# sash-a/CleanRL.jl

Hardware: NVIDIA B200
Metric: ppo_env_steps_per_sec (higher is better)
Workload: dtype f32

## Files before the change

### cleanrl.jl_b200/csrc/rollout.cu

```cuda
#include "kernels.h"
#include "mlp_tile.cuh"

namespace {

constexpr int RE = 32;
constexpr int ROLL_FWD = CRL_THREADS;
constexpr int ROLL_THREADS = ROLL_FWD + 64;
constexpr int BIG_FWD = 128, BIG_THREADS = BIG_FWD + 64;
constexpr int BAR_FWD = 1, BAR_SPEC = 2, BAR_BOOK = 3;

__device__ __forceinline__ void nbar_sync(int id, int n) { asm volatile("bar.sync %0, %1;" ::"r"(id), "r"(n) : "memory"); }
__device__ __forceinline__ void nbar_arrive(int id, int n) { asm volatile("bar.arrive %0, %1;" ::"r"(id), "r"(n) : "memory"); }

template <int ENV> struct RolloutSmem {
  using G = TileGeom<4, 2>;
  using E = EnvTraits<ENV>;
  static constexpr int SP = G::S_PAD;
  static constexpr int PARAMS = 0;
  static constexpr int X = PARAMS + SmemParams<ENV>::SIZE;
  static constexpr int H1 = X + CRL_MAXD * SP;
  static constexpr int H2 = H1 + G::ROWS * SP;
  static constexpr int OUT = H2 + G::ROWS * SP;
  static constexpr int ST = OUT + 4 * RE;
  static constexpr int SPEC = ST + 4 * RE;
  static constexpr int RST = SPEC + 2 * 4 * RE;
  static constexpr int NOISE = RST + 4 * RE;
  static constexpr int USED = NOISE + 2 * RE;
  static constexpr int BOOK = USED + RE;
  static constexpr int FLOATS = BOOK + 4 * RE;
  static constexpr size_t BYTES = FLOATS * sizeof(float);
  static_assert((NOISE % 2) == 0, "the Float64 uniforms need 8-byte alignment");
};

#ifdef ROLL_TRACE
#define RTR(i) do { if (tr) tr[i] = clock64(); } while (0)
#else
#define RTR(i) do { } while (0)
#endif

template <int ENV> struct HeadRow { float w[CRL_H]; float b; };
template <int ENV> __device__ __forceinline__ void load_head_row(const float* sp, HeadRow<ENV>& hr) {
  using E = EnvTraits<ENV>;
  const int o = threadIdx.x / RE;
#pragma unroll
  for (int k = 0; k < CRL_H; k++) hr.w[k] = 0.0f;
  hr.b = 0.0f;
  if (threadIdx.x >= RE * (E::A + 1)) return;
  if (o < E::A) {
    const float* a = sp + SmemParams<ENV>::ACTOR;
#pragma unroll
    for (int k = 0; k < CRL_H; k++) hr.w[k] = a[NetOff<E::D, E::A>::W3 + k * E::A + o];
    hr.b = a[NetOff<E::D, E::A>::B3 + o];
  } else {
    const float* c = sp + SmemParams<ENV>::CRITIC;
#pragma unroll
    for (int k = 0; k < CRL_H; k++) hr.w[k] = c[NetOff<E::D, 1>::W3 + k];
    hr.b = c[NetOff<E::D, 1>::B3];
  }
}

template <int ENV, bool BOOKSYNC = false>
__device__ __forceinline__ void forward32(const ThreadCoord<TileGeom<4, 2>>& tc, float* smem, const HeadRow<ENV>& hr,
                                          long long* tr = nullptr) {
  using G = TileGeom<4, 2>;
  using E = EnvTraits<ENV>;
  using SM = RolloutSmem<ENV>;
  constexpr int SP = G::S_PAD;
  float* sp = smem + SM::PARAMS;
  float* xs = smem + SM::X;
  float* h1 = smem + SM::H1;
  float* h2 = smem + SM::H2;
  float* so = smem + SM::OUT;
  const float* np = sp + net_base<ENV>(tc.net);
  using NO = NetOff<E::D, 1>;
  RTR(0);
  tile_layer_fwd4<G, E::D>(tc, np + NO::W1, np + NO::B1, xs, h1 + tc.net * CRL_H * SP);
  RTR(1);
  nbar_sync(BAR_FWD, ROLL_FWD);
  RTR(2);
  tile_layer_fwd4<G, CRL_H>(tc, np + NO::W2, np + NO::B2, h1 + tc.net * CRL_H * SP, h2 + tc.net * CRL_H * SP);
  RTR(3);
  nbar_sync(BAR_FWD, ROLL_FWD);
  RTR(4);
  if (threadIdx.x < RE * (E::A + 1)) {
    const int o = threadIdx.x / RE, e = threadIdx.x % RE;
    const float* hrow = h2 + (o < E::A ? 0 : CRL_H) * SP + e;
    float hv[CRL_H];
#pragma unroll
    for (int k = 0; k < CRL_H; k++) hv[k] = hrow[k * SP];
    if (BOOKSYNC) nbar_sync(BAR_BOOK, RE * (E::A + 1) + 32);
    float acc = 0.0f;
#pragma unroll
    for (int k = 0; k < CRL_H; k++) acc = fmaf(hr.w[k], hv[k], acc);
    acc += hr.b;
    so[o * RE + e] = acc;
  }
  RTR(5);
  nbar_sync(BAR_FWD, ROLL_FWD);
  RTR(6);
}

struct FwdCoord8x4 {
  int q, p, net, nb;
  __device__ FwdCoord8x4() {
    const int lane = threadIdx.x & 31, w = (threadIdx.x >> 5) & 3;
    q = w * 4 + (lane >> 3);
    p = lane & 7;
    net = q >> 3;
    nb = 8 * (q & 7);
  }
};
template <int K>
__device__ __forceinline__ void fwd_layer_8x4(const FwdCoord8x4& fc, const float* __restrict__ Wt, const float* __restrict__ bias,
                                              const float* __restrict__ in, float* __restrict__ out) {
  constexpr int SP = RE + 4, PF = 2;
  const float* wp = Wt + fc.nb;
  const float* ap = in + 4 * fc.p;
  const float4 b0 = *reinterpret_cast<const float4*>(bias + fc.nb), b1 = *reinterpret_cast<const float4*>(bias + fc.nb + 4);
  float2 acc[8][2];
#pragma unroll
  for (int j = 0; j < 8; j++) acc[j][0] = acc[j][1] = make_float2(0.0f, 0.0f);
  float4 w0[PF], w1[PF], av[PF];
#pragma unroll
  for (int i = 0; i < PF; i++) {
    if (i < K) {
      w0[i] = *reinterpret_cast<const float4*>(wp + i * CRL_H);
      w1[i] = *reinterpret_cast<const float4*>(wp + i * CRL_H + 4);
      av[i] = *reinterpret_cast<const float4*>(ap + i * SP);
    }
  }
#pragma unroll
  for (int k0 = 0; k0 < K; k0 += PF) {
    float4 w0n[PF], w1n[PF], avn[PF];
#pragma unroll
    for (int i = 0; i < PF; i++) {
      if (k0 + PF + i < K) {
        w0n[i] = *reinterpret_cast<const float4*>(wp + (k0 + PF + i) * CRL_H);
        w1n[i] = *reinterpret_cast<const float4*>(wp + (k0 + PF + i) * CRL_H + 4);
        avn[i] = *reinterpret_cast<const float4*>(ap + (k0 + PF + i) * SP);
      }
    }
#pragma unroll
    for (int i = 0; i < PF; i++) {
      if (k0 + i < K) {
        const float2 a01 = make_float2(av[i].x, av[i].y), a23 = make_float2(av[i].z, av[i].w);
#pragma unroll
        for (int j = 0; j < 8; j++) {
          const float wj = j < 4 ? f4_get(w0[i], j) : f4_get(w1[i], j - 4);
          const float2 ww = make_float2(wj, wj);
          acc[j][0] = __ffma2_rn(ww, a01, acc[j][0]);
          acc[j][1] = __ffma2_rn(ww, a23, acc[j][1]);
        }
      }
    }
#pragma unroll
    for (int i = 0; i < PF; i++) { w0[i] = w0n[i]; w1[i] = w1n[i]; av[i] = avn[i]; }
  }
#pragma unroll
  for (int j = 0; j < 8; j++) {
    const float b = j < 4 ? f4_get(b0, j) : f4_get(b1, j - 4);
    const float2 t0 = tanh_fast2(__fadd2_rn(acc[j][0], make_float2(b, b)));
    const float2 t1 = tanh_fast2(__fadd2_rn(acc[j][1], make_float2(b, b)));
    *reinterpret_cast<float4*>(out + (fc.nb + j) * SP + 4 * fc.p) = make_float4(t0.x, t0.y, t1.x, t1.y);
  }
}
template <int ENV>
__device__ __forceinline__ void forward32_big(const FwdCoord8x4& fc, float* smem) {
  using E = EnvTraits<ENV>;
  using SM = RolloutSmem<ENV>;
  constexpr int SP = RE + 4;
  static_assert(SP == TileGeom<4, 2>::S_PAD, "both forward variants share one activation layout");
  float* sp = smem + SM::PARAMS;
  float* xs = smem + SM::X;
  float* h1 = smem + SM::H1;
  float* h2 = smem + SM::H2;
  float* so = smem + SM::OUT;
  const float* np = sp + net_base<ENV>(fc.net);
  using NO = NetOff<E::D, 1>;
  fwd_layer_8x4<E::D>(fc, np + NO::W1, np + NO::B1, xs, h1 + fc.net * CRL_H * SP);
  nbar_sync(BAR_FWD, BIG_FWD);
  fwd_layer_8x4<CRL_H>(fc, np + NO::W2, np + NO::B2, h1 + fc.net * CRL_H * SP, h2 + fc.net * CRL_H * SP);
  nbar_sync(BAR_FWD, BIG_FWD);
  if (threadIdx.x < RE * (E::A + 1)) {
    const int o = threadIdx.x / RE, e = threadIdx.x % RE;
    const float* hrow = h2 + (o < E::A ? 0 : CRL_H) * SP + e;
    nbar_sync(BAR_BOOK, RE * (E::A + 1) + 32);
    float acc = 0.0f;
    if (o < E::A) {
      const float* a = sp + SmemParams<ENV>::ACTOR;
#pragma unroll 16
      for (int k = 0; k < CRL_H; k++) acc = fmaf(a[NetOff<E::D, E::A>::W3 + k * E::A + o], hrow[k * SP], acc);
      acc += a[NetOff<E::D, E::A>::B3 + o];
    } else {
      const float* c = sp + SmemParams<ENV>::CRITIC;
#pragma unroll 16
      for (int k = 0; k < CRL_H; k++) acc = fmaf(c[NetOff<E::D, 1>::W3 + k], hrow[k * SP], acc);
      acc += c[NetOff<E::D, 1>::B3];
    }
    so[o * RE + e] = acc;
  }
  nbar_sync(BAR_FWD, BIG_FWD);
}

template <int ENV, bool BIG>
__global__ void __launch_bounds__(BIG ? BIG_THREADS : ROLL_THREADS, BIG ? 2 : 1) rollout_kernel(RolloutArgs a) {
  constexpr int FWD = BIG ? BIG_FWD : ROLL_FWD;
  constexpr int SW0 = FWD / 32;
  using G = TileGeom<4, 2>;
  using E = EnvTraits<ENV>;
  using SM = RolloutSmem<ENV>;
  constexpr int SP = G::S_PAD;
  constexpr int D = E::D, A = E::A, S = E::S;
  constexpr bool CART = ENV == CRL_ENV_CARTPOLE;
  extern __shared__ __align__(16) float smem[];
  float* sp = smem + SM::PARAMS;
  float* xs = smem + SM::X;
  float* so = smem + SM::OUT;
  float* st_s = smem + SM::ST;
  float* spec_s = smem + SM::SPEC;
  float* rst_s = smem + SM::RST;
  double* noise_d = reinterpret_cast<double*>(smem + SM::NOISE);
  float* noise_f = smem + SM::NOISE;
  int* used_s = reinterpret_cast<int*>(smem + SM::USED);
  int* act_s = reinterpret_cast<int*>(smem + SM::BOOK);
  float* actf_s = smem + SM::BOOK + RE;
  float* rew_s = smem + SM::BOOK + 2 * RE;
  int* done_s = reinterpret_cast<int*>(smem + SM::BOOK + 3 * RE);
  const ThreadCoord<G> tc;
  const FwdCoord8x4 fc;

  load_params<ENV>(a.params, sp);
  for (int i = threadIdx.x; i < CRL_MAXD * SP; i += blockDim.x) xs[i] = 0.0f;

  const int warp = threadIdx.x >> 5;
  const int e = threadIdx.x & 31;
  const long long n = (long long)blockIdx.x * RE + e;
  const bool fwd = threadIdx.x < FWD;
  const bool owner = threadIdx.x < RE;
  const bool booker = warp == SW0 + 1;
  const bool in_range = n < a.N;
  const bool valid = owner && in_range;
  const unsigned long long step0 = a.ds->policy_step;
  const uint32_t gid = (uint32_t)(a.env_id_base + (int)n);

  float st[S];
  float obs[D];
  int env_t = 0;
  uint32_t resets = 0;
  bool done_flag = false;
  int ep_len = 0;
  double ep_ret = 0.0;
  bool prev_done = false;
  float obs_b[D];
  unsigned long long agg_n = 0;
  double agg_ret = 0.0, agg_len = 0.0, agg_max = -INFINITY;
  bool rec_pending = false;
  unsigned int rec_slot = 0;
  crl_episode rec;
  rec.step = 0; rec.env = 0; rec.length = 0; rec._pad = 0; rec.episode_return = 0.0;

#pragma unroll
  for (int i = 0; i < S; i++) st[i] = 0.0f;
#pragma unroll
  for (int k = 0; k < D; k++) obs_b[k] = 0.0f;
  if (valid) {
#pragma unroll
    for (int i = 0; i < S; i++) st[i] = a.env_state[n * S + i];
    env_t = a.env_t[n];
    resets = a.reset_count[n];
  }
  if (booker && in_range) {
    ep_len = a.ep_length[n];
    ep_ret = a.ep_return[n];
    resets = a.reset_count[n];
  }
  __syncthreads();
  HeadRow<ENV> hr;
  if (!BIG) load_head_row<ENV>(sp, hr);
  if (owner) {
    env_obs<ENV>(st, obs);
#pragma unroll
    for (int k = 0; k < D; k++) xs[k * SP + e] = obs[k];
#pragma unroll
    for (int i = 0; i < S; i++) st_s[i * RE + e] = st[i];
    used_s[e] = 0;
  }
  auto prepare_reset = [&]() {
    float u4[4], rs[S];
    int rt;
    rng_reset_uniforms(a.seed, gid, resets, u4);
    env_reset<ENV>(rs, rt, u4);
#pragma unroll
    for (int i = 0; i < S; i++) rst_s[i * RE + e] = rs[i];
  };
  if (booker && !a.reset_noise) prepare_reset();

  auto book = [&](int tb, const float (&zv)[A + 1], int act_i, float act_f, float r, bool dn) {
    const long long b = (long long)tb * a.N + n;
    ep_len += 1;
    float logprob;
    if (!E::CONT) {
      float m = zv[0];
#pragma unroll
      for (int k = 1; k < A; k++) m = fmaxf(m, zv[k]);
      float sum = 0.0f;
#pragma unroll
      for (int k = 0; k < A; k++) sum = __fadd_rn(sum, expf(__fsub_rn(zv[k], m)));
      const float ls = logf(sum);
      logprob = __fsub_rn(__fsub_rn(zv[0], m), ls);
#pragma unroll
      for (int k = 1; k < A; k++) logprob = (act_i == k) ? __fsub_rn(__fsub_rn(zv[k], m), ls) : logprob;
    } else {
      float lps = 0.0f;
#pragma unroll
      for (int k = 0; k < A; k++) {
        const float mean = zv[k];
        const float logstd = sp[SmemParams<ENV>::LOGSTD + k];
        const float sd = expf(logstd);
        const float diff = __fsub_rn(act_f, mean);
        const float q = __fdiv_rn(-__fmul_rn(diff, diff), __fmul_rn(__fmul_rn(2.0f, sd), sd));
        lps = __fadd_rn(lps, __fsub_rn(__fsub_rn(q, logstd), 0.9189385332046727f));
      }
      logprob = lps;
    }
    if (rec_pending) {
      if (rec_slot < (unsigned int)a.ep_capacity) a.records[rec_slot] = rec;
      rec_pending = false;
    }
    ep_ret += (double)r;
    if (in_range) {
      if (D == 4) {
        reinterpret_cast<float4*>(a.state)[b] = make_float4(obs_b[0], obs_b[1], obs_b[2], obs_b[3]);
      } else {
#pragma unroll
        for (int k = 0; k < D; k++) a.state[b * D + k] = obs_b[k];
      }
      if (!E::CONT) reinterpret_cast<int32_t*>(a.action)[b] = act_i;
      else reinterpret_cast<float*>(a.action)[b * A] = act_f;
      a.logprob[b] = logprob;
      a.value[b] = zv[A];
      a.terminal[b] = prev_done ? 1 : 0;
      a.reward[b] = r;
      if (dn) {
        rec_slot = atomicAdd(&a.eb->count, 1u);
        rec_pending = true;
        rec.step = tb; rec.env = (int)n; rec.length = ep_len; rec._pad = 0; rec.episode_return = ep_ret;
        agg_n += 1; agg_ret += ep_ret; agg_len += (double)ep_len; agg_max = fmax(agg_max, ep_ret);
        ep_ret = 0.0;
        ep_len = 0;
      }
    }
    prev_done = dn;
  };
  static_assert(!E::CONT || A == 1, "the Gaussian head hands one action per env to the bookkeeping warp");
  __syncthreads();

  for (int t = 0; t < a.T; t++) {
    if (!fwd) {
      if (booker) {
        float zv[A + 1];
#pragma unroll
        for (int k = 0; k <= A; k++) zv[k] = so[k * RE + e];
        const int act_i = act_s[e];
        const float act_f = actf_s[e], r = rew_s[e];
        const bool dn = done_s[e] != 0;
        nbar_arrive(BAR_BOOK, RE * (A + 1) + 32);
        if (t > 0) book(t - 1, zv, act_i, act_f, r, dn);
#pragma unroll
        for (int k = 0; k < D; k++) obs_b[k] = xs[k * SP + e];
        if (!a.reset_noise && used_s[e]) {
          resets += 1;
          prepare_reset();
          used_s[e] = 0;
        }
      }
      if (warp == SW0 && !a.action_noise) {
        if (!E::CONT) {
          noise_d[e] = in_range ? rng_action_uniform(a.seed, gid, step0 + (unsigned long long)t) : 0.0;
        } else {
          float zn[2] = {0.0f, 0.0f};
          if (in_range) rng_action_normals(a.seed, gid, step0 + (unsigned long long)t, zn);
          noise_f[e] = zn[0];
          noise_f[RE + e] = zn[1];
        }
      }
      if (CART) {
        float s4[4];
#pragma unroll
        for (int i = 0; i < 4; i++) s4[i] = st_s[i * RE + e];
        cartpole_dynamics(s4, warp - SW0);
#pragma unroll
        for (int i = 0; i < 4; i++) spec_s[((warp - SW0) * 4 + i) * RE + e] = s4[i];
      }
      __threadfence_block();
      nbar_arrive(BAR_SPEC, RE + 64);
    } else {
      if (BIG) forward32_big<ENV>(fc, smem); else forward32<ENV, true>(tc, smem, hr);
      if (owner) {
        const long long b = (long long)t * a.N + n;
        int act_i = 0;
        float act_f = 0.0f;
        if (!E::CONT) {
          float z[A], p[A];
#pragma unroll
          for (int k = 0; k < A; k++) z[k] = so[k * RE + e];
          float m = z[0];
#pragma unroll
          for (int k = 1; k < A; k++) m = fmaxf(m, z[k]);
          float ex[A], sum = 0.0f;
#pragma unroll
          for (int k = 0; k < A; k++) { ex[k] = expf(__fsub_rn(z[k], m)); sum = __fadd_rn(sum, ex[k]); }
          float psum = 0.0f;
#pragma unroll
          for (int k = 0; k < A; k++) {
            p[k] = __fdiv_rn(ex[k], sum);
            psum = __fadd_rn(psum, p[k]);
          }
          nbar_sync(BAR_SPEC, RE + 64);
          double u = 0.0;
          if (valid) u = a.action_noise ? a.action_noise[b] : noise_d[e];
          const double tt = __dmul_rn(u, (double)psum);
          float cw = p[0];
          int i = 0;
#pragma unroll
          for (int k = 1; k < A; k++) {
            if ((double)cw < tt && i == k - 1) { i = k; cw = __fadd_rn(cw, p[k]); }
          }
          act_i = i;
        } else {
          nbar_sync(BAR_SPEC, RE + 64);
          float zn = 0.0f;
          if (valid) zn = a.action_noise ? (float)a.action_noise[b * A] : noise_f[e];
          const float mean = so[e];
          const float sd = expf(sp[SmemParams<ENV>::LOGSTD]);
          act_f = __fadd_rn(mean, __fmul_rn(sd, zn));
        }
        float r;
        bool dn;
        if (CART) {
#pragma unroll
          for (int i = 0; i < 4; i++) st[i] = spec_s[(act_i * 4 + i) * RE + e];
          env_t += 1;
          cartpole_outcome(st, env_t, a.max_steps, r, dn);
        } else {
          pendulum_step(st, env_t, act_f, a.max_steps, r, dn);
        }
        env_obs<ENV>(st, obs);
        done_flag = dn;
        act_s[e] = act_i; actf_s[e] = act_f; rew_s[e] = r; done_s[e] = dn ? 1 : 0;
        if (valid && dn) {
          if (a.reset_noise) {
            const float4 v = reinterpret_cast<const float4*>(a.reset_noise)[b];
            const float u4[4] = {v.x, v.y, v.z, v.w};
            env_reset<ENV>(st, env_t, u4);
          } else {
#pragma unroll
            for (int i = 0; i < S; i++) st[i] = rst_s[i * RE + e];
            env_t = 0;
            used_s[e] = 1;
          }
          resets += 1;
          if (a.fresh_obs_after_reset) env_obs<ENV>(st, obs);
        }
#pragma unroll
        for (int k = 0; k < D; k++) xs[k * SP + e] = obs[k];
#pragma unroll
        for (int i = 0; i < S; i++) st_s[i * RE + e] = st[i];
      }
    }
    __syncthreads();
  }
  if (!fwd) {
    if (booker) {
      float zv[A + 1];
#pragma unroll
      for (int k = 0; k <= A; k++) zv[k] = so[k * RE + e];
      const int act_i = act_s[e];
      const float act_f = actf_s[e], r = rew_s[e];
      const bool dn = done_s[e] != 0;
      nbar_arrive(BAR_BOOK, RE * (A + 1) + 32);
      book(a.T - 1, zv, act_i, act_f, r, dn);
      if (rec_pending && rec_slot < (unsigned int)a.ep_capacity) a.records[rec_slot] = rec;
      if (in_range) {
        a.ep_length[n] = ep_len;
        a.ep_return[n] = ep_ret;
      }
      const double sr = warp_sum(agg_ret), sl = warp_sum(agg_len), mx = warp_max(agg_max);
      unsigned long long cn = agg_n;
#pragma unroll
      for (int o = 16; o > 0; o >>= 1) cn += __shfl_xor_sync(0xffffffffu, cn, o);
      if (e == 0 && cn > 0) {
        atomicAdd(&a.eb->n_episodes, cn);
        atomicAdd(&a.eb->sum_return, sr);
        atomicAdd(&a.eb->sum_length, sl);
        unsigned long long* addr = reinterpret_cast<unsigned long long*>(&a.eb->max_return);
        unsigned long long old = *addr, assumed;
        do {
          assumed = old;
          if (__longlong_as_double((long long)assumed) >= mx) break;
          old = atomicCAS(addr, assumed, (unsigned long long)__double_as_longlong(mx));
        } while (assumed != old);
      }
    }
    return;
  }

  float obs_last[D];
#pragma unroll
  for (int k = 0; k < D; k++) obs_last[k] = obs[k];
  if (owner) {
    float fresh[D];
    env_obs<ENV>(st, fresh);
#pragma unroll
    for (int k = 0; k < D; k++) xs[k * SP + e] = fresh[k];
  }
  nbar_sync(BAR_FWD, FWD);
  if (BIG) forward32_big<ENV>(fc, smem); else forward32<ENV, true>(tc, smem, hr);
  if (valid) {
    a.next_value[n] = so[A * RE + e];
#pragma unroll
    for (int i = 0; i < S; i++) a.env_state[n * S + i] = st[i];
    a.env_t[n] = env_t;
    a.reset_count[n] = resets;
#pragma unroll
    for (int k = 0; k < D; k++) a.next_obs[n * D + k] = obs_last[k];
    a.next_done[n] = done_flag ? 1 : 0;
  }
}

template <int ENV>
__global__ void env_step_raw_kernel(float* state, int* t, const void* action, float* reward, uint8_t* done,
                                    long long n, int max_steps) {
  constexpr int S = EnvTraits<ENV>::S;
  const long long i = (long long)blockIdx.x * blockDim.x + threadIdx.x;
  if (i >= n) return;
  float st[S];
#pragma unroll
  for (int k = 0; k < S; k++) st[k] = state[i * S + k];
  int tt = t[i];
  float r;
  bool dn;
  if (ENV == CRL_ENV_CARTPOLE) cartpole_step(st, tt, reinterpret_cast<const int32_t*>(action)[i], max_steps, r, dn);
  else pendulum_step(st, tt, reinterpret_cast<const float*>(action)[i], max_steps, r, dn);
#pragma unroll
  for (int k = 0; k < S; k++) state[i * S + k] = st[k];
  t[i] = tt;
  reward[i] = r;
  done[i] = dn ? 1 : 0;
}

template <int ENV>
__global__ void __launch_bounds__(CRL_THREADS) policy_forward_raw_kernel(const float* params, const float* obs,
                                                                         float* out_policy, float* logp,
                                                                         float* value, long long n) {
  using G = TileGeom<4, 2>;
  using E = EnvTraits<ENV>;
  using SM = RolloutSmem<ENV>;
  constexpr int SP = G::S_PAD;
  constexpr int D = E::D, A = E::A;
  extern __shared__ __align__(16) float smem[];
  float* xs = smem + SM::X;
  float* so = smem + SM::OUT;
  const ThreadCoord<G> tc;
  load_params<ENV>(params, smem + SM::PARAMS);
  const int e = threadIdx.x;
  const long long i = (long long)blockIdx.x * RE + e;
  if (e < RE) {
#pragma unroll
    for (int k = 0; k < D; k++) xs[k * SP + e] = i < n ? obs[i * D + k] : 0.0f;
  }
  __syncthreads();
  HeadRow<ENV> hr;
  load_head_row<ENV>(smem + SM::PARAMS, hr);
  forward32<ENV>(tc, smem, hr);
  if (e < RE && i < n) {
    float z[A];
#pragma unroll
    for (int k = 0; k < A; k++) { z[k] = so[k * RE + e]; out_policy[i * A + k] = z[k]; }
    value[i] = so[A * RE + e];
    if (!E::CONT) {
      float m = z[0];
#pragma unroll
      for (int k = 1; k < A; k++) m = fmaxf(m, z[k]);
      float sum = 0.0f;
#pragma unroll
      for (int k = 0; k < A; k++) sum = __fadd_rn(sum, expf(__fsub_rn(z[k], m)));
      const float ls = logf(sum);
#pragma unroll
      for (int k = 0; k < A; k++) logp[i * A + k] = __fsub_rn(__fsub_rn(z[k], m), ls);
    }
  }
}

template <int ENV> cudaError_t launch_rollout_t(const RolloutArgs& a, cudaStream_t s) {
  const int grid = (a.N + RE - 1) / RE;
  static int sms = 0;
  if (sms == 0) {
    int dev = 0;
    cudaGetDevice(&dev);
    cudaDeviceGetAttribute(&sms, cudaDevAttrMultiProcessorCount, dev);
  }
  if (grid > sms) rollout_kernel<ENV, true><<<grid, BIG_THREADS, RolloutSmem<ENV>::BYTES, s>>>(a);
  else rollout_kernel<ENV, false><<<grid, ROLL_THREADS, RolloutSmem<ENV>::BYTES, s>>>(a);
  return cudaGetLastError();
}

template <int ENV>
cudaError_t launch_policy_forward_t(const float* params, const float* obs, float* out_policy, float* logp,
                                    float* value, long long n, cudaStream_t s) {
  const long long grid = (n + RE - 1) / RE;
  if (grid == 0) return cudaSuccess;
  policy_forward_raw_kernel<ENV><<<(unsigned)grid, CRL_THREADS, RolloutSmem<ENV>::BYTES, s>>>(params, obs, out_policy,
                                                                                              logp, value, n);
  return cudaGetLastError();
}

__global__ void episode_buf_init_kernel(EpisodeBuf* eb) {
  eb->count = 0; eb->_pad = 0; eb->n_episodes = 0ull; eb->sum_return = 0.0; eb->sum_length = 0.0;
  eb->max_return = -INFINITY;
}

template <int ENV> cudaError_t init_attrs_t() {
  cudaError_t e = cudaFuncSetAttribute(rollout_kernel<ENV, false>, cudaFuncAttributeMaxDynamicSharedMemorySize,
                                       (int)RolloutSmem<ENV>::BYTES);
  if (e != cudaSuccess) return e;
  e = cudaFuncSetAttribute(rollout_kernel<ENV, true>, cudaFuncAttributeMaxDynamicSharedMemorySize, (int)RolloutSmem<ENV>::BYTES);
  if (e != cudaSuccess) return e;
  return cudaFuncSetAttribute(policy_forward_raw_kernel<ENV>, cudaFuncAttributeMaxDynamicSharedMemorySize,
                              (int)RolloutSmem<ENV>::BYTES);
}

}

cudaError_t kernels_init_rollout() {
  cudaError_t e = init_attrs_t<CRL_ENV_CARTPOLE>();
  if (e != cudaSuccess) return e;
  return init_attrs_t<CRL_ENV_PENDULUM>();
}

cudaError_t launch_episode_buf_init(EpisodeBuf* eb, cudaStream_t s) {
  episode_buf_init_kernel<<<1, 1, 0, s>>>(eb);
  return cudaGetLastError();
}

cudaError_t launch_rollout(int env_kind, const RolloutArgs& a, cudaStream_t s) {
  return env_kind == CRL_ENV_CARTPOLE ? launch_rollout_t<CRL_ENV_CARTPOLE>(a, s) : launch_rollout_t<CRL_ENV_PENDULUM>(a, s);
}

cudaError_t launch_env_step_raw(int env_kind, float* state, int* t, const void* action, float* reward,
                                uint8_t* done, long long n, int max_steps, cudaStream_t s) {
  if (n == 0) return cudaSuccess;
  const unsigned grid = (unsigned)((n + 127) / 128);
  if (env_kind == CRL_ENV_CARTPOLE)
    env_step_raw_kernel<CRL_ENV_CARTPOLE><<<grid, 128, 0, s>>>(state, t, action, reward, done, n, max_steps);
  else
    env_step_raw_kernel<CRL_ENV_PENDULUM><<<grid, 128, 0, s>>>(state, t, action, reward, done, n, max_steps);
  return cudaGetLastError();
}

cudaError_t launch_policy_forward_raw(int env_kind, const float* params, const float* obs, float* out_policy,
                                      float* logp, float* value, long long n, cudaStream_t s) {
  return env_kind == CRL_ENV_CARTPOLE
             ? launch_policy_forward_t<CRL_ENV_CARTPOLE>(params, obs, out_policy, logp, value, n, s)
             : launch_policy_forward_t<CRL_ENV_PENDULUM>(params, obs, out_policy, logp, value, n, s);
}

namespace {
template <int ENV>
__global__ void env_reset_kernel(int N, unsigned long long seed, int env_id_base, float* env_state, int* env_t,
                                 double* ep_return, int* ep_length, uint32_t* reset_count, float* next_obs,
                                 uint8_t* next_done) {
  constexpr int S = EnvTraits<ENV>::S, D = EnvTraits<ENV>::D;
  const int n = blockIdx.x * blockDim.x + threadIdx.x;
  if (n >= N) return;
  float u4[4], st[S], obs[D];
  const uint32_t k = reset_count[n];
  rng_reset_uniforms(seed, (uint32_t)(env_id_base + n), k, u4);
  int t;
  env_reset<ENV>(st, t, u4);
  env_obs<ENV>(st, obs);
#pragma unroll
  for (int i = 0; i < S; i++) env_state[n * S + i] = st[i];
#pragma unroll
  for (int i = 0; i < D; i++) next_obs[n * D + i] = obs[i];
  env_t[n] = t;
  reset_count[n] = k + 1;
  next_done[n] = 0;
  ep_return[n] = 0.0;
  ep_length[n] = 0;
}
template <int ENV>
__global__ void env_refresh_kernel(int N, const float* env_state, float* next_obs, uint8_t* next_done) {
  constexpr int S = EnvTraits<ENV>::S, D = EnvTraits<ENV>::D;
  const int n = blockIdx.x * blockDim.x + threadIdx.x;
  if (n >= N) return;
  float st[S], obs[D];
#pragma unroll
  for (int i = 0; i < S; i++) st[i] = env_state[n * S + i];
  env_obs<ENV>(st, obs);
#pragma unroll
  for (int i = 0; i < D; i++) next_obs[n * D + i] = obs[i];
  next_done[n] = 0;
}
}

cudaError_t launch_env_reset(int env_kind, int N, unsigned long long seed, int env_id_base, float* env_state,
                             int* env_t, double* ep_return, int* ep_length, uint32_t* reset_count, float* next_obs,
                             uint8_t* next_done, cudaStream_t s) {
  const int grid = (N + 127) / 128;
  if (env_kind == CRL_ENV_CARTPOLE)
    env_reset_kernel<CRL_ENV_CARTPOLE><<<grid, 128, 0, s>>>(N, seed, env_id_base, env_state, env_t, ep_return, ep_length,
                                                           reset_count, next_obs, next_done);
  else
    env_reset_kernel<CRL_ENV_PENDULUM><<<grid, 128, 0, s>>>(N, seed, env_id_base, env_state, env_t, ep_return, ep_length,
                                                           reset_count, next_obs, next_done);
  return cudaGetLastError();
}

cudaError_t launch_env_refresh(int env_kind, int N, const float* env_state, float* next_obs, uint8_t* next_done,
                               cudaStream_t s) {
  const int grid = (N + 127) / 128;
  if (env_kind == CRL_ENV_CARTPOLE) env_refresh_kernel<CRL_ENV_CARTPOLE><<<grid, 128, 0, s>>>(N, env_state, next_obs, next_done);
  else env_refresh_kernel<CRL_ENV_PENDULUM><<<grid, 128, 0, s>>>(N, env_state, next_obs, next_done);
  return cudaGetLastError();
}
```

Baseline: 249.1 million.

## Move critic evaluation out of rollout loop into separate batched value pass

The rollout kernel now runs only the actor network per step and no longer computes values or the final bootstrap forward. The forward thread counts are halved because only one network is evaluated. A new value_pass_kernel runs afterwards over all stored states plus the final env states, computing the critic per thread with weights in shared memory and packed FMAs. The intent is to take the critic off the serial per-step critical path and run it fully in parallel, at the cost of an extra launch and re-reading the stored observations.

```diff
diff --git a/cleanrl.jl_b200/csrc/rollout.cu b/cleanrl.jl_b200/csrc/rollout.cu
--- a/cleanrl.jl_b200/csrc/rollout.cu
+++ b/cleanrl.jl_b200/csrc/rollout.cu
@@ -1,12 +1,14 @@
 #include "kernels.h"
 #include "mlp_tile.cuh"
 
+#include <algorithm>
+
 namespace {
 
 constexpr int RE = 32;
-constexpr int ROLL_FWD = CRL_THREADS;
+constexpr int ROLL_FWD = 128;
 constexpr int ROLL_THREADS = ROLL_FWD + 64;
-constexpr int BIG_FWD = 128, BIG_THREADS = BIG_FWD + 64;
+constexpr int BIG_FWD = 64, BIG_THREADS = BIG_FWD + 64;
 constexpr int BAR_FWD = 1, BAR_SPEC = 2, BAR_BOOK = 3;
 
 __device__ __forceinline__ void nbar_sync(int id, int n) { asm volatile("bar.sync %0, %1;" ::"r"(id), "r"(n) : "memory"); }
@@ -39,13 +41,13 @@
 #endif
 
 template <int ENV> struct HeadRow { float w[CRL_H]; float b; };
-template <int ENV> __device__ __forceinline__ void load_head_row(const float* sp, HeadRow<ENV>& hr) {
+template <int ENV, bool CRITIC> __device__ __forceinline__ void load_head_row(const float* sp, HeadRow<ENV>& hr) {
   using E = EnvTraits<ENV>;
   const int o = threadIdx.x / RE;
 #pragma unroll
   for (int k = 0; k < CRL_H; k++) hr.w[k] = 0.0f;
   hr.b = 0.0f;
-  if (threadIdx.x >= RE * (E::A + 1)) return;
+  if (threadIdx.x >= RE * (E::A + (CRITIC ? 1 : 0))) return;
   if (o < E::A) {
     const float* a = sp + SmemParams<ENV>::ACTOR;
 #pragma unroll
@@ -59,13 +61,14 @@
   }
 }
 
-template <int ENV, bool BOOKSYNC = false>
+template <int ENV, bool CRITIC>
 __device__ __forceinline__ void forward32(const ThreadCoord<TileGeom<4, 2>>& tc, float* smem, const HeadRow<ENV>& hr,
                                           long long* tr = nullptr) {
   using G = TileGeom<4, 2>;
   using E = EnvTraits<ENV>;
   using SM = RolloutSmem<ENV>;
   constexpr int SP = G::S_PAD;
+  constexpr int NFWD = CRITIC ? CRL_THREADS : ROLL_FWD, HEADS = E::A + (CRITIC ? 1 : 0);
   float* sp = smem + SM::PARAMS;
   float* xs = smem + SM::X;
   float* h1 = smem + SM::H1;
@@ -76,19 +79,19 @@
   RTR(0);
   tile_layer_fwd4<G, E::D>(tc, np + NO::W1, np + NO::B1, xs, h1 + tc.net * CRL_H * SP);
   RTR(1);
-  nbar_sync(BAR_FWD, ROLL_FWD);
+  nbar_sync(BAR_FWD, NFWD);
   RTR(2);
   tile_layer_fwd4<G, CRL_H>(tc, np + NO::W2, np + NO::B2, h1 + tc.net * CRL_H * SP, h2 + tc.net * CRL_H * SP);
   RTR(3);
-  nbar_sync(BAR_FWD, ROLL_FWD);
+  nbar_sync(BAR_FWD, NFWD);
   RTR(4);
-  if (threadIdx.x < RE * (E::A + 1)) {
+  if (threadIdx.x < RE * HEADS) {
     const int o = threadIdx.x / RE, e = threadIdx.x % RE;
     const float* hrow = h2 + (o < E::A ? 0 : CRL_H) * SP + e;
     float hv[CRL_H];
 #pragma unroll
     for (int k = 0; k < CRL_H; k++) hv[k] = hrow[k * SP];
-    if (BOOKSYNC) nbar_sync(BAR_BOOK, RE * (E::A + 1) + 32);
+    if (!CRITIC) nbar_sync(BAR_BOOK, RE * HEADS + 32);
     float acc = 0.0f;
 #pragma unroll
     for (int k = 0; k < CRL_H; k++) acc = fmaf(hr.w[k], hv[k], acc);
@@ -96,7 +99,7 @@
     so[o * RE + e] = acc;
   }
   RTR(5);
-  nbar_sync(BAR_FWD, ROLL_FWD);
+  nbar_sync(BAR_FWD, NFWD);
   RTR(6);
 }
 
@@ -170,33 +173,26 @@
   using SM = RolloutSmem<ENV>;
   constexpr int SP = RE + 4;
   static_assert(SP == TileGeom<4, 2>::S_PAD, "both forward variants share one activation layout");
+  static_assert(BIG_FWD == 64, "two warps of 8 x 4 tiles cover the actor's 64 neurons x 32 envs");
   float* sp = smem + SM::PARAMS;
   float* xs = smem + SM::X;
   float* h1 = smem + SM::H1;
   float* h2 = smem + SM::H2;
   float* so = smem + SM::OUT;
-  const float* np = sp + net_base<ENV>(fc.net);
+  const float* np = sp + SmemParams<ENV>::ACTOR;
   using NO = NetOff<E::D, 1>;
-  fwd_layer_8x4<E::D>(fc, np + NO::W1, np + NO::B1, xs, h1 + fc.net * CRL_H * SP);
+  fwd_layer_8x4<E::D>(fc, np + NO::W1, np + NO::B1, xs, h1);
   nbar_sync(BAR_FWD, BIG_FWD);
-  fwd_layer_8x4<CRL_H>(fc, np + NO::W2, np + NO::B2, h1 + fc.net * CRL_H * SP, h2 + fc.net * CRL_H * SP);
+  fwd_layer_8x4<CRL_H>(fc, np + NO::W2, np + NO::B2, h1, h2);
   nbar_sync(BAR_FWD, BIG_FWD);
-  if (threadIdx.x < RE * (E::A + 1)) {
+  if (threadIdx.x < RE * E::A) {
     const int o = threadIdx.x / RE, e = threadIdx.x % RE;
-    const float* hrow = h2 + (o < E::A ? 0 : CRL_H) * SP + e;
-    nbar_sync(BAR_BOOK, RE * (E::A + 1) + 32);
+    const float* hrow = h2 + e;
+    nbar_sync(BAR_BOOK, RE * E::A + 32);
     float acc = 0.0f;
-    if (o < E::A) {
-      const float* a = sp + SmemParams<ENV>::ACTOR;
 #pragma unroll 16
-      for (int k = 0; k < CRL_H; k++) acc = fmaf(a[NetOff<E::D, E::A>::W3 + k * E::A + o], hrow[k * SP], acc);
-      acc += a[NetOff<E::D, E::A>::B3 + o];
-    } else {
-      const float* c = sp + SmemParams<ENV>::CRITIC;
-#pragma unroll 16
-      for (int k = 0; k < CRL_H; k++) acc = fmaf(c[NetOff<E::D, 1>::W3 + k], hrow[k * SP], acc);
-      acc += c[NetOff<E::D, 1>::B3];
-    }
+    for (int k = 0; k < CRL_H; k++) acc = fmaf(np[NetOff<E::D, E::A>::W3 + k * E::A + o], hrow[k * SP], acc);
+    acc += np[NetOff<E::D, E::A>::B3 + o];
     so[o * RE + e] = acc;
   }
   nbar_sync(BAR_FWD, BIG_FWD);
@@ -276,7 +272,7 @@
   }
   __syncthreads();
   HeadRow<ENV> hr;
-  if (!BIG) load_head_row<ENV>(sp, hr);
+  if (!BIG) load_head_row<ENV, false>(sp, hr);
   if (owner) {
     env_obs<ENV>(st, obs);
 #pragma unroll
@@ -295,7 +291,7 @@
   };
   if (booker && !a.reset_noise) prepare_reset();
 
-  auto book = [&](int tb, const float (&zv)[A + 1], int act_i, float act_f, float r, bool dn) {
+  auto book = [&](int tb, const float (&zv)[A], int act_i, float act_f, float r, bool dn) {
     const long long b = (long long)tb * a.N + n;
     ep_len += 1;
     float logprob;
@@ -338,7 +334,6 @@
       if (!E::CONT) reinterpret_cast<int32_t*>(a.action)[b] = act_i;
       else reinterpret_cast<float*>(a.action)[b * A] = act_f;
       a.logprob[b] = logprob;
-      a.value[b] = zv[A];
       a.terminal[b] = prev_done ? 1 : 0;
       a.reward[b] = r;
       if (dn) {
@@ -358,13 +353,13 @@
   for (int t = 0; t < a.T; t++) {
     if (!fwd) {
       if (booker) {
-        float zv[A + 1];
-#pragma unroll
-        for (int k = 0; k <= A; k++) zv[k] = so[k * RE + e];
+        float zv[A];
+#pragma unroll
+        for (int k = 0; k < A; k++) zv[k] = so[k * RE + e];
         const int act_i = act_s[e];
         const float act_f = actf_s[e], r = rew_s[e];
         const bool dn = done_s[e] != 0;
-        nbar_arrive(BAR_BOOK, RE * (A + 1) + 32);
+        nbar_arrive(BAR_BOOK, RE * A + 32);
         if (t > 0) book(t - 1, zv, act_i, act_f, r, dn);
 #pragma unroll
         for (int k = 0; k < D; k++) obs_b[k] = xs[k * SP + e];
@@ -395,7 +390,7 @@
       __threadfence_block();
       nbar_arrive(BAR_SPEC, RE + 64);
     } else {
-      if (BIG) forward32_big<ENV>(fc, smem); else forward32<ENV, true>(tc, smem, hr);
+      if (BIG) forward32_big<ENV>(fc, smem); else forward32<ENV, false>(tc, smem, hr);
       if (owner) {
         const long long b = (long long)t * a.N + n;
         int act_i = 0;
@@ -472,14 +467,10 @@
   }
   if (!fwd) {
     if (booker) {
-      float zv[A + 1];
-#pragma unroll
-      for (int k = 0; k <= A; k++) zv[k] = so[k * RE + e];
-      const int act_i = act_s[e];
-      const float act_f = actf_s[e], r = rew_s[e];
-      const bool dn = done_s[e] != 0;
-      nbar_arrive(BAR_BOOK, RE * (A + 1) + 32);
-      book(a.T - 1, zv, act_i, act_f, r, dn);
+      float zv[A];
+#pragma unroll
+      for (int k = 0; k < A; k++) zv[k] = so[k * RE + e];
+      book(a.T - 1, zv, act_s[e], actf_s[e], rew_s[e], done_s[e] != 0);
       if (rec_pending && rec_slot < (unsigned int)a.ep_capacity) a.records[rec_slot] = rec;
       if (in_range) {
         a.ep_length[n] = ep_len;
@@ -505,25 +496,13 @@
     return;
   }
 
-  float obs_last[D];
-#pragma unroll
-  for (int k = 0; k < D; k++) obs_last[k] = obs[k];
-  if (owner) {
-    float fresh[D];
-    env_obs<ENV>(st, fresh);
-#pragma unroll
-    for (int k = 0; k < D; k++) xs[k * SP + e] = fresh[k];
-  }
-  nbar_sync(BAR_FWD, FWD);
-  if (BIG) forward32_big<ENV>(fc, smem); else forward32<ENV, true>(tc, smem, hr);
   if (valid) {
-    a.next_value[n] = so[A * RE + e];
 #pragma unroll
     for (int i = 0; i < S; i++) a.env_state[n * S + i] = st[i];
     a.env_t[n] = env_t;
     a.reset_count[n] = resets;
 #pragma unroll
-    for (int k = 0; k < D; k++) a.next_obs[n * D + k] = obs_last[k];
+    for (int k = 0; k < D; k++) a.next_obs[n * D + k] = obs[k];
     a.next_done[n] = done_flag ? 1 : 0;
   }
 }
@@ -571,8 +550,8 @@
   }
   __syncthreads();
   HeadRow<ENV> hr;
-  load_head_row<ENV>(smem + SM::PARAMS, hr);
-  forward32<ENV>(tc, smem, hr);
+  load_head_row<ENV, true>(smem + SM::PARAMS, hr);
+  forward32<ENV, true>(tc, smem, hr);
   if (e < RE && i < n) {
     float z[A];
 #pragma unroll
@@ -592,16 +571,107 @@
   }
 }
 
+constexpr int VP_THREADS = 128, VP_J = 16;
+template <int ENV>
+__global__ void __launch_bounds__(VP_THREADS, 4) value_pass_kernel(const float* __restrict__ params,
+                                                                const float* __restrict__ state,
+                                                                const float* __restrict__ env_state,
+                                                                float* __restrict__ value, float* __restrict__ next_value,
+                                                                long long TN, int N) {
+  using E = EnvTraits<ENV>;
+  using NO = NetOff<E::D, 1>;
+  constexpr int D = E::D, S = E::S;
+  static_assert(NO::B1 % 4 == 0 && NO::W2 % 4 == 0 && NO::B2 % 4 == 0 && NO::W3 % 4 == 0, "float4 weight loads");
+  __shared__ __align__(16) float w[(NO::SIZE + 3) & ~3];
+  for (int i = threadIdx.x; i < NO::SIZE; i += VP_THREADS) w[i] = params[E::NET_A + i];
+  __syncthreads();
+  const long long total = TN + N;
+  for (long long i = (long long)blockIdx.x * VP_THREADS + threadIdx.x; i < total; i += (long long)gridDim.x * VP_THREADS) {
+    float x[D];
+    if (i < TN) {
+      if constexpr (D == 4) {
+        const float4 v = reinterpret_cast<const float4*>(state)[i];
+        x[0] = v.x; x[1] = v.y; x[2] = v.z; x[3] = v.w;
+      } else {
+#pragma unroll
+        for (int k = 0; k < D; k++) x[k] = state[i * D + k];
+      }
+    } else {
+      float st[S];
+#pragma unroll
+      for (int k = 0; k < S; k++) st[k] = env_state[(i - TN) * S + k];
+      env_obs<ENV>(st, x);
+    }
+    float h1[CRL_H];
+#pragma unroll
+    for (int j0 = 0; j0 < CRL_H; j0 += 4) {
+      float2 a01 = make_float2(0.0f, 0.0f), a23 = a01;
+#pragma unroll
+      for (int k = 0; k < D; k++) {
+        const float4 wk = *reinterpret_cast<const float4*>(w + NO::W1 + k * CRL_H + j0);
+        a01 = __ffma2_rn(make_float2(wk.x, wk.y), f2s(x[k]), a01);
+        a23 = __ffma2_rn(make_float2(wk.z, wk.w), f2s(x[k]), a23);
+      }
+      const float4 b = *reinterpret_cast<const float4*>(w + NO::B1 + j0);
+      const float2 t01 = tanh_fast2(__fadd2_rn(a01, make_float2(b.x, b.y)));
+      const float2 t23 = tanh_fast2(__fadd2_rn(a23, make_float2(b.z, b.w)));
+      h1[j0] = t01.x; h1[j0 + 1] = t01.y; h1[j0 + 2] = t23.x; h1[j0 + 3] = t23.y;
+    }
+    float v = 0.0f;
+#pragma unroll 1
+    for (int j0 = 0; j0 < CRL_H; j0 += VP_J) {
+      float2 acc[VP_J / 2];
+#pragma unroll
+      for (int j = 0; j < VP_J / 2; j++) acc[j] = make_float2(0.0f, 0.0f);
+#pragma unroll
+      for (int k = 0; k < CRL_H; k++) {
+        const float2 hk = f2s(h1[k]);
+#pragma unroll
+        for (int c = 0; c < VP_J / 4; c++) {
+          const float4 wk = *reinterpret_cast<const float4*>(w + NO::W2 + k * CRL_H + j0 + 4 * c);
+          acc[2 * c] = __ffma2_rn(make_float2(wk.x, wk.y), hk, acc[2 * c]);
+          acc[2 * c + 1] = __ffma2_rn(make_float2(wk.z, wk.w), hk, acc[2 * c + 1]);
+        }
+      }
+#pragma unroll
+      for (int c = 0; c < VP_J / 4; c++) {
+        const float4 b = *reinterpret_cast<const float4*>(w + NO::B2 + j0 + 4 * c);
+        const float4 w3 = *reinterpret_cast<const float4*>(w + NO::W3 + j0 + 4 * c);
+        const float2 t01 = tanh_fast2(__fadd2_rn(acc[2 * c], make_float2(b.x, b.y)));
+        const float2 t23 = tanh_fast2(__fadd2_rn(acc[2 * c + 1], make_float2(b.z, b.w)));
+        v = fmaf(w3.x, t01.x, v);
+        v = fmaf(w3.y, t01.y, v);
+        v = fmaf(w3.z, t23.x, v);
+        v = fmaf(w3.w, t23.y, v);
+      }
+    }
+    v += w[NO::B3];
+    if (i < TN) value[i] = v;
+    else next_value[i - TN] = v;
+  }
+}
+
 template <int ENV> cudaError_t launch_rollout_t(const RolloutArgs& a, cudaStream_t s) {
   const int grid = (a.N + RE - 1) / RE;
-  static int sms = 0;
+  static int sms = 0, vp_ctas = 0;
   if (sms == 0) {
     int dev = 0;
     cudaGetDevice(&dev);
     cudaDeviceGetAttribute(&sms, cudaDevAttrMultiProcessorCount, dev);
   }
+  if (vp_ctas == 0) {
+    int per_sm = 0;
+    cudaOccupancyMaxActiveBlocksPerMultiprocessor(&per_sm, value_pass_kernel<ENV>, VP_THREADS, 0);
+    vp_ctas = sms * std::max(per_sm, 1);
+  }
   if (grid > sms) rollout_kernel<ENV, true><<<grid, BIG_THREADS, RolloutSmem<ENV>::BYTES, s>>>(a);
   else rollout_kernel<ENV, false><<<grid, ROLL_THREADS, RolloutSmem<ENV>::BYTES, s>>>(a);
+  cudaError_t e = cudaGetLastError();
+  if (e != cudaSuccess) return e;
+  const long long TN = (long long)a.T * a.N, total = TN + a.N;
+  const int vgrid = (int)std::min<long long>(vp_ctas, (total + VP_THREADS - 1) / VP_THREADS);
+  if (vgrid == 0) return cudaSuccess;
+  value_pass_kernel<ENV><<<vgrid, VP_THREADS, 0, s>>>(a.params, a.state, a.env_state, a.value, a.next_value, TN, a.N);
   return cudaGetLastError();
 }
 
```

New measurement: 252.3 million, median of 6. 1.01x the previous value.
